# Kiripiro/leaffliction

Hardware: AMD Instinct MI355X
Metric: 224x224 images/sec train (higher is better)
Workload: dtype f32; 1 GPU; leaf_cnn base train step (configs[1]: img 224, batch 256/GPU, fp32, 8 classes, AdamW+clipnorm+EMA, in-model augmentation); per_gpu_batch=256, global_batch=256, img_size=224, parallelism=dp1

## Files before the change

### include/leafhip.h

```cpp
#ifndef LEAFHIP_H
#define LEAFHIP_H

#include <stddef.h>
#include <stdint.h>

#ifdef __cplusplus
extern "C" {
#endif

#define LF_OK 0
#define LF_ERR_INVALID (-1)
#define LF_ERR_LAUNCH (-2)
#define LF_ERR_WORKSPACE (-3)

#define LF_VERSION 100

typedef void* lf_stream_t;

int lf_version(void);
const char* lf_last_error(void);

int lf_copy_rows(void* dst, size_t dst_pitch, const void* src, size_t src_pitch, size_t width, size_t rows, int to_host,
                 lf_stream_t stream);

// ... 296 lines not shown
                        int accumulate, int mask, int* out);
int lf_conv2d_wgrad_bf16_plan(int n, int cin, int h, int w, int cout, int ksize, int* out);

long long lf_conv2d_stats_tiles(int n, int cin, int h, int w, int cout, int ksize);
int lf_conv2d_stats_f32(const float* x, const float* w, float* y, int n, int cin, int h, int wd,
                        int cout, int ksize, const float* in_scale, const float* in_shift,
                        int in_relu, const float* pivot, float* tile_part, size_t tile_part_bytes,
                        lf_stream_t stream, const float* wino_u);

int lf_conv2d_bnbwd_f32(const float* x, const float* w, float* y, int n, int cin, int h, int wd,
                        int cout, int ksize, int accumulate, const float* mask_y,
                        const float* mask_scale, const float* mask_shift, int mask_relu,
                        float* tile_part, size_t tile_part_bytes, lf_stream_t stream, const float* wino_u);

int lf_conv2d_dgrad_weights_f32(const float* w, float* wt, int cin, int ksize, int cout,
                                lf_stream_t stream);

int lf_conv2d_takes_wino_filters(int cin, int h, int wd, int cout, int ksize);
int lf_conv2d_wino_filters_f32(const float* w, float* u, int cin, int cout, int dgrad, lf_stream_t stream);

size_t lf_conv2d_wgrad_workspace(int n, int cin, int h, int wd, int cout, int ksize);
int lf_conv2d_wgrad_f32(const float* x, const float* dy, int n, int cin, int h, int wd, int cout,
                        int ksize, const float* in_scale, const float* in_shift, int in_relu,
                        void* workspace, size_t ws_bytes, lf_stream_t stream);
int lf_conv2d_wgrad_reduce_f32(void* workspace, float* dw, int n, int cin, int h, int wd,
                               int cout, int ksize, float beta, lf_stream_t stream);
int lf_conv2d_wgrad_bn_supported(int n, int cin, int h, int w, int cout, int ksize);
int lf_conv2d_wgrad_bn_f32(const float* x, const float* g, const float* bn_y,
                           const float* alpha_nc, const float* add_nc, const float* coef,
                           int bn_relu, float* dy_out, int n, int cin, int h, int w, int cout,
                           int ksize, const float* in_scale, const float* in_shift, int in_relu,
                           void* workspace, size_t ws_bytes, lf_stream_t stream);

int lf_dwconv3x3_f32(const float* x, const float* w, float* y, int n, int c, int h, int wd,
                     const float* in_scale, const float* in_shift, int in_relu, lf_stream_t stream);
size_t lf_dwconv3x3_bwd_workspace(int n, int c, int h, int wd);
int lf_dwconv3x3_bwd_f32(const float* x, const float* w, const float* dy, float* dx, int accumulate, float* dw,
                         int n, int c, int h, int wd, const float* in_scale, const float* in_shift, int in_relu,
                         void* workspace, size_t ws_bytes, lf_stream_t stream);

int lf_head_distill_fwd_f32(const float* feat, const float* w, const float* b, const float* ytrue,
                            const float* tprobs, float temperature, float alpha, float* probs, float* soft,
                            float* loss, float* kd, int n, int f, int c, lf_stream_t stream);
int lf_head_distill_bwd_f32(const float* feat, const float* w, const float* probs, const float* ytrue,
                            const float* soft, float temperature, float alpha, float* dlogits, float* dfeat,
                            float* dw, float* db, int n, int f, int c, float inv_n, lf_stream_t stream);

int lf_input_stage_f32(const uint8_t* in, float* out, int n, int h, int w, const float* aug4,
                       const float* mean3, const float* denom3, float* means_ws,
                       lf_stream_t stream);

int lf_scale_shift_act_f32(const float* x, float* out, int n, int c, int hw, const float* scale,
                           const float* shift, int relu, lf_stream_t stream);
size_t lf_bn_workspace(int c);
int lf_bn_train_stats_f32(const float* y, int n, int c, int hw, const float* gamma,
                          const float* beta, float* moving_mean, float* moving_var, float momentum,
                          float eps, float* mean, float* invstd, float* scale, float* shift,
                          void* workspace, size_t ws_bytes, lf_stream_t stream);
int lf_bn_train_stats_tiles_f32(const float* tile_part, long long tiles, int n, int c, int hw,
                                const float* gamma, const float* beta, float* moving_mean,
                                float* moving_var, float momentum, float eps, float* mean,
                                float* invstd, float* scale, float* shift, void* workspace,
                                size_t ws_bytes, lf_stream_t stream);
int lf_bn_infer_scale_shift_f32(int c, const float* gamma, const float* beta,
                                const float* moving_mean, const float* moving_var, float eps,
                                float* scale, float* shift, lf_stream_t stream);
// ... 60 lines not shown
```

### leaffliction_amd/_lib.py

```python
from __future__ import annotations

import ctypes as C
import os
from pathlib import Path

_LIB = None

LIB_PATH = Path(__file__).resolve().parent / "libleafhip.so"

c_void_p, c_int, c_size_t, c_u64, c_float, c_double = (
    C.c_void_p, C.c_int, C.c_size_t, C.c_uint64, C.c_float, C.c_double)
P = c_void_p

SIGNATURES = {
    "lf_version": [],
    "lf_last_error": [],
    "lf_pack_hwc_u8_to_nchw_f32": [P, P, c_int, c_int, c_int, P, P, P],
    "lf_hist_u8": [P, P, c_int, c_int, c_int, P],
    "lf_autocontrast_lut": [P, P, P, c_int, P],
    "lf_lut_apply_u8": [P, P, P, c_int, c_int, c_int, P],
    "lf_gather_rows_u8": [P, P, P, c_int, c_size_t, P],
    "lf_flip_u8": [P, P, P, c_int, c_int, c_int, P],
    "lf_noise_wrap_add_u8": [P, P, P, c_size_t, P],
    "lf_add_wrap_u8": [P, P, P, c_size_t, P],
# ... 79 lines not shown
    "lf_canvas_tiles_u8": [P, c_int, c_int, c_int, P, P, c_size_t, c_int, c_int, c_int, P],
    "lf_hist_figure_u8": [P, P, P, c_int, P],
    "lf_conv2d_bf16_stats_tiles": [c_int, c_int, c_int, c_int, c_int, c_int, c_int],
    "lf_conv2d_bf16_train": [P, c_int, P, P, c_int, c_int, c_int, c_int, c_int, c_int, P, P, c_int, c_int, P,
                             c_size_t, P, P, P, P, c_int, P],
    "lf_conv2d_wgrad_bf16_workspace": [c_int, c_int, c_int, c_int, c_int, c_int],
    "lf_conv2d_wgrad_bf16": [P, P, P, P, P, P, c_int, P, P, c_int, c_int, c_int, c_int, c_int, c_int, P, P,
                             c_int, P, c_size_t, P],
    "lf_gap_stats_bf16": [P, P, P, c_int, c_int, c_int, P, P, c_int, P],
    "lf_block_tail_fwd_train_bf16": [P, P, P, P, P, P, P, c_int, P, P, P, c_int, c_int, c_int, c_int, P],
    "lf_block_tail_bwd_bf16": [P, P, P, P, P, P, P, P, P, P, P, c_int, c_int, c_int, c_int, P],
    "lf_bcast_planes_bf16": [P, P, c_int, c_int, c_float, P],
    "lf_cast_f32_bf16": [P, P, c_size_t, P],
    "lf_cast_bf16_f32": [P, P, c_size_t, P],
    "lf_conv2d_variant": [c_int, c_int, c_int, c_int],
    "lf_conv2d_wgrad_variant": [c_int, c_int, c_int, c_int, c_int, c_int],
    "lf_conv2d_plan": [c_int, c_int, c_int, c_int, c_int, c_int, P],
    "lf_conv2d_wgrad_plan": [c_int, c_int, c_int, c_int, c_int, c_int, P],
    "lf_conv2d_bf16_plan": [c_int, c_int, c_int, c_int, c_int, c_int, c_int, c_int, c_int, c_int, c_int, P],
    "lf_conv2d_wgrad_bf16_plan": [c_int, c_int, c_int, c_int, c_int, c_int, P],
    "lf_conv2d_stats_tiles": [c_int, c_int, c_int, c_int, c_int, c_int],
    "lf_conv2d_stats_f32": [P, P, P, c_int, c_int, c_int, c_int, c_int, c_int, P, P, c_int, P, P, c_size_t, P, P],
    "lf_conv2d_bnbwd_f32": [P, P, P, c_int, c_int, c_int, c_int, c_int, c_int, c_int, P, P, P, c_int, P,
                            c_size_t, P, P],
    "lf_conv2d_dgrad_weights_f32": [P, P, c_int, c_int, c_int, P],
    "lf_conv2d_takes_wino_filters": [c_int, c_int, c_int, c_int, c_int],
    "lf_conv2d_wino_filters_f32": [P, P, c_int, c_int, c_int, P],
    "lf_conv2d_wgrad_workspace": [c_int, c_int, c_int, c_int, c_int, c_int],
    "lf_conv2d_wgrad_f32": [P, P, c_int, c_int, c_int, c_int, c_int, c_int, P, P, c_int, P,
                            c_size_t, P],
    "lf_conv2d_wgrad_bn_supported": [c_int, c_int, c_int, c_int, c_int, c_int],
    "lf_conv2d_wgrad_bn_f32": [P, P, P, P, P, P, c_int, P, c_int, c_int, c_int, c_int, c_int, c_int, P, P,
                               c_int, P, c_size_t, P],
    "lf_dwconv3x3_f32": [P, P, P, c_int, c_int, c_int, c_int, P, P, c_int, P],
    "lf_dwconv3x3_bwd_workspace": [c_int, c_int, c_int, c_int],
    "lf_dwconv3x3_bwd_f32": [P, P, P, P, c_int, P, c_int, c_int, c_int, c_int, P, P, c_int, P, c_size_t, P],
    "lf_conv2d_wgrad_reduce_f32": [P, P, c_int, c_int, c_int, c_int, c_int, c_int, c_float, P],
    "lf_input_stage_f32": [P, P, c_int, c_int, c_int, P, P, P, P, P],
    "lf_scale_shift_act_f32": [P, P, c_int, c_int, c_int, P, P, c_int, P],
    "lf_bn_workspace": [c_int],
    "lf_bn_train_stats_f32": [P, c_int, c_int, c_int, P, P, P, P, c_float, c_float, P, P, P, P,
                              P, c_size_t, P],
    "lf_bn_train_stats_tiles_f32": [P, C.c_longlong, c_int, c_int, c_int, P, P, P, P, c_float, c_float, P, P, P, P, P, c_size_t, P],
    "lf_bn_bwd_sums_f32": [P, P, P, P, P, P, P, P, c_int, P, P, P, P, P, P, c_int, c_int, c_int, P,
                           c_size_t, P],
    "lf_bn_bwd_sums_tiles_f32": [P, C.c_longlong, P, P, P, P, P, P, P, P, c_int, c_int, c_int, P,
                                 c_size_t, P],
    "lf_bn_infer_scale_shift_f32": [c_int, P, P, P, P, c_float, P, P, P],
    "lf_bn_bwd_f32": [P, P, P, P, P, P, P, P, c_int, P, P, P, P, P, P, c_int, c_int, c_int, c_int, P,
                      c_size_t, P],
    "lf_gap_f32": [P, P, c_int, c_int, c_int, P, P, c_int, P, P],
    "lf_bcast_planes_f32": [P, P, c_int, c_int, c_float, P],
    "lf_se_fwd_f32": [P, P, P, P, P, P, P, c_int, c_int, c_int, P],
    "lf_se_bwd_workspace": [c_int, c_int, c_int],
    "lf_se_bwd_f32": [P, P, P, P, P, P, P, P, P, P, P, c_int, c_int, c_int, c_float, P, c_size_t, P],
    "lf_block_tail_fwd_f32": [P, P, P, P, P, P, P, c_int, P, P, P, c_int, c_int, c_int, c_int, P],
    "lf_block_tail_bwd_f32": [P, P, P, P, P, P, P, P, P, P, P, c_int, c_int, c_int, c_int, P],
    "lf_head_fwd_f32": [P, P, P, P, P, P, c_int, c_int, c_int, P],
    "lf_head_bwd_f32": [P, P, P, P, P, P, P, P, c_int, c_int, c_int, c_float, P],
    "lf_head_distill_fwd_f32": [P, P, P, P, P, c_float, c_float, P, P, P, P, c_int, c_int, c_int, P],
    "lf_head_distill_bwd_f32": [P, P, P, P, P, c_float, c_float, P, P, P, P, c_int, c_int, c_int, c_float, P],
    "lf_mul_f32": [P, P, P, c_size_t, P],
    "lf_adamw_workspace": [c_int],
    "lf_adamw_step_f32": [P, P, P, P, P, P, P, c_int, C.c_longlong, c_float, c_float, c_float,
                          c_float, c_float, c_float, C.c_longlong, c_float, c_int, P, P, c_size_t, P],
    "lf_ema_update_f32": [P, P, c_size_t, c_float, c_int, P],
}
_RESTYPES = {"lf_last_error": C.c_char_p, "lf_conv2d_wgrad_workspace": c_size_t,
             "lf_dwconv3x3_bwd_workspace": c_size_t,
             "lf_bn_workspace": c_size_t, "lf_se_bwd_workspace": c_size_t,
             "lf_adamw_workspace": c_size_t, "lf_conv2d_stats_tiles": C.c_longlong,
             "lf_blur_saliency_workspace": c_size_t, "lf_inclusive_mask_workspace": c_size_t, "lf_make_mask_workspace": c_size_t, "lf_brown_spots_workspace": c_size_t, "lf_lesion_table_workspace": c_size_t, "lf_canny_workspace": c_size_t, "lf_clahe_workspace": c_size_t,
             "lf_good_features_workspace": c_size_t, "lf_landmarks_workspace": c_size_t,
             "lf_conv2d_bf16_weight_elems": c_size_t,
             "lf_conv2d_bf16_act_mean_workspace": c_size_t,
             "lf_conv2d_bf16_stats_tiles": C.c_longlong, "lf_conv2d_wgrad_bf16_workspace": c_size_t,
             "lf_jpeg_file_bound": c_size_t, "lf_jpeg_scan_aux_offset": c_size_t, "lf_jpeg_scan_aux_offset_ragged": c_size_t, "lf_jpeg_decode_items_workspace": c_size_t, "lf_jpeg_entropy_workspace": c_size_t, "lf_jpeg_wrap_scan": C.c_long, "lf_jpeg_fdct_groups": C.c_long, "lf_jpeg_decode_workspace": c_size_t, "lf_jpeg_write_file": C.c_long, "lf_jpeg_quant_tables": None}


class ResampleItem(C.Structure):
    _fields_ = [("in_off", C.c_int64), ("tile_start", C.c_int64), ("h", C.c_int32), ("w", C.c_int32),
                ("out_index", C.c_int32), ("xtab", C.c_int32), ("ytab", C.c_int32), ("kx", C.c_int32),
                ("ky", C.c_int32), ("reserved", C.c_int32)]


class LeafHipError(RuntimeError):
    pass


def load():
    global _LIB
    if _LIB is not None:
        return _LIB
    import torch
    path = Path(os.environ.get("LEAFHIP_LIB", LIB_PATH))
    if not path.exists():
        raise LeafHipError(
            f"{path} not found: build it with `python -c 'import __graft_entry__ as g; g.build()'` "
            "or `make -C leaffliction_amd/csrc` (there is no CPU fallback)")
    lib = C.CDLL(str(path))
    for name, argtypes in SIGNATURES.items():
# ... 18 lines not shown
```

### leaffliction_amd/csrc/lf_conv.hip

```cpp
#include <type_traits>

#include "lf_common.h"

namespace {

typedef float f32x16 __attribute__((ext_vector_type(16)));
typedef float f32x4 __attribute__((ext_vector_type(4)));

constexpr int kThreads = 256;

typedef float lf_f4 __attribute__((ext_vector_type(4)));
constexpr unsigned kBufOob = 0xffffffffu;
__device__ __forceinline__ __amdgpu_buffer_rsrc_t buf_rsrc(const float* base, unsigned bytes) {
    return __builtin_amdgcn_make_buffer_rsrc(const_cast<float*>(base), 0, bytes, 0x00020000);
}
__device__ __forceinline__ float4 buf_load4(__amdgpu_buffer_rsrc_t r, unsigned off) {
    const lf_f4 v = __builtin_bit_cast(lf_f4, __builtin_amdgcn_raw_buffer_load_b128(r, off, 0, 0));
    return make_float4(v.x, v.y, v.z, v.w);
}
__device__ __forceinline__ float buf_load1(__amdgpu_buffer_rsrc_t r, unsigned off) {
    return __builtin_bit_cast(float, __builtin_amdgcn_raw_buffer_load_b32(r, off, 0, 0));
}

struct ConvArgs {
// ... 733 lines not shown
    if (__all(y2 && lane_full && co0 + CT <= p.cout))
        epilogue(std::true_type{});
    else
        epilogue(std::false_type{});
    if (stats) write_stat_part<WPX, CT>(p, red, t.bz, t.tile, co0, tid);
}

struct WgradArgs {
    const float* x;
    const float* dy;
    float* part;
    const float* in_scale;
    const float* in_shift;
    int n, cin, cout, h, wd;
    int tiles_x, tiles_y, items, items_per_split;
    int in_relu;
    int vec_ok;
    const float* bn_y;
    const float* bn_alpha;
    const float* bn_add;
    const float* bn_coef;
    float* dy_out;
    int bn_relu;
};

__device__ __forceinline__ float bn_dy1(float g, float y, float al, float ad, float c0, float c1,
                                        float c2, float c3, float c4, int relu) {
    float dz = fmaf(g, al, ad);
    if (relu && !(fmaf(y, c0, c1) > 0.f)) dz = 0.f;
    return fmaf(c2, dz, fmaf(c3, y, c4));
}

template <int TW, int TH, int WCI, int WCO, int KSPL>
__global__ __launch_bounds__(kThreads, 4) void wgrad_mfma_kernel(WgradArgs p) {
    static_assert(WCI * WCO * KSPL == 4, "wave decomposition");
    static_assert(TH % KSPL == 0 && TW % 4 == 0, "rows split across waves, float4 rows");
    constexpr int PP = (TW * TH) | 1;
    constexpr int CI_T = 32 * WCI, CO_T = 32 * WCO;
    constexpr int XSZ = CI_T * PP, DSZ = CO_T * PP;
    constexpr int RED = KSPL > 1 ? 1024 : 0;
    constexpr int LDSF = XSZ + DSZ > RED ? XSZ + DSZ : RED;
    constexpr int TW4 = TW / 4;
    constexpr int NXI = CI_T * TH * TW4, XPT = (NXI + kThreads - 1) / kThreads;
    constexpr int NDI = CO_T * TH * TW4, DPT = (NDI + kThreads - 1) / kThreads;
    __shared__ float lds[LDSF];
    float* lx = lds;
    float* ld = lds + XSZ;

    const int tid = threadIdx.x, lane = tid & 63, wid = tid >> 6;
    const int w_ci = wid % WCI, w_co = (wid / WCI) % WCO, w_k = wid / (WCI * WCO);
    const lf::Block3 blk = lf::xcd_split_block3();
    const int ci0 = blk.y * CI_T, co0 = blk.z * CO_T;
    const int khalf = lane >> 5, j = lane & 31;
    const size_t hw = (size_t)p.h * p.wd;
    const unsigned uhw = (unsigned)hw;

    f32x16 acc;
#pragma unroll
    for (int r = 0; r < 16; ++r) acc[r] = 0.f;

    const int abase = (w_ci * 32 + j) * PP + khalf;
    const int bbase = (w_co * 32 + j) * PP + khalf;
    const bool pro = p.in_scale != nullptr;

    auto compute_item = [&]() {
        constexpr int ROWS = TH / KSPL;
#pragma unroll
// ... 202 lines not shown
        }
    }

    if (KSPL > 1) {
        const int q = w_co * WCI + w_ci;
#pragma unroll 1
        for (int k = 1; k < KSPL; ++k) {
#pragma unroll 1
            for (int qq = 0; qq < WCI * WCO; ++qq) {
                __syncthreads();
                if (w_k == k && q == qq) {
#pragma unroll
                    for (int r = 0; r < 16; ++r) lds[r * 64 + lane] = acc[r];
                }
                __syncthreads();
                if (w_k == 0 && q == qq) {
#pragma unroll
                    for (int r = 0; r < 16; ++r) acc[r] += lds[r * 64 + lane];
                }
            }
        }
    }
    if (w_k == 0) {
        float* out = p.part + (size_t)blk.x * p.cin * p.cout;
        const int co = co0 + w_co * 32 + j;
#pragma unroll
        for (int r = 0; r < 16; ++r) {
            const int ci = ci0 + w_ci * 32 + (r & 3) + 8 * (r >> 2) + 4 * khalf;
            if (ci < p.cin && co < p.cout) out[(size_t)ci * p.cout + co] = acc[r];
        }
    }
}


template <int TW, int TH, int WCI, int WCO, int KSPL>
constexpr int wgrad3_lds_floats() {
    const int pp = ((TW + 2) * (TH + 2)) | 1, dp = (TW * TH) | 1;
    const int buf = 32 * WCI * pp + 32 * WCO * dp;
    const int red = KSPL > 1 ? 16 * 1024 : 0;
    const int xch = WCI * WCO * 2 * 3 * 1024;
    const int m = 2 * buf > red ? 2 * buf : red;
    return m > xch ? m : xch;
}

template <int TW, int TH, int WCI, int WCO, int KSPL>
__global__ __launch_bounds__(64 * 2 * WCI * WCO * KSPL, 2) void wgrad3_kernel(WgradArgs p) {
    constexpr int NT = 64 * 2 * WCI * WCO * KSPL;
    constexpr int TWH = TW / 2, NTILE = TWH * (TH / 2), SH = NTILE / KSPL;
    static_assert(TH % 2 == 0 && TW % 4 == 0 && NTILE % KSPL == 0 && SH % 2 == 0,
                  "2x2 tiles split across waves in pairs, float4 rows");
    static_assert(SH % TWH == 0 || TWH % SH == 0, "a K-split share is whole tile rows or part of one");
    constexpr int PW = TW + 2, PH = TH + 2;
    constexpr int PP = (PW * PH) | 1;
    constexpr int DP = (TW * TH) | 1;
    constexpr int CI_T = 32 * WCI, CO_T = 32 * WCO, NQ = WCI * WCO;
    constexpr int XSZ = CI_T * PP, DSZ = CO_T * DP;
    constexpr int BUF = XSZ + DSZ;
    static_assert(wgrad3_lds_floats<TW, TH, WCI, WCO, KSPL>() >= 2 * BUF, "LDS sizing");
    constexpr int TW4 = TW / 4;
    constexpr int NXI = CI_T * PH * TW4, XPT = (NXI + NT - 1) / NT;
    constexpr int NHI = CI_T * PH * 2 * 1, HPT = (NHI + NT - 1) / NT;
    constexpr int NDI = CO_T * TH * TW4, DPT = (NDI + NT - 1) / NT;
    extern __shared__ __attribute__((aligned(16))) float lds[];

    const int tid = threadIdx.x, lane = tid & 63, wid = tid >> 6;
    const int pg = wid & 1, rest = wid >> 1;
// ... 654 lines not shown
        best.tiles_x = (w + 31) / 32;
        best.tiles_y = (h + 7) / 8;
        best.gy = 1;
        best.gz = (cout + 31) / 32;
    } else {
        long long best_cost = -1;
        for (int v = 0; v < (int)(sizeof(kWgVariants) / sizeof(kWgVariants[0])); ++v) {
            const WgVariant& k = kWgVariants[v];
            const long long tx = (w + k.tw - 1) / k.tw, ty = (h + k.th - 1) / k.th;
            const long long gy = (cin + k.ci_t - 1) / k.ci_t, gz = (cout + k.co_t - 1) / k.co_t;
            const long long cost = tx * k.tw * ty * k.th * gy * k.ci_t * gz * k.co_t;
            if (best_cost < 0 || cost < best_cost) {
                best_cost = cost;
                best.variant = v;
                best.tw = k.tw;
                best.tiles_x = (int)tx;
                best.tiles_y = (int)ty;
                best.gy = (int)gy;
                best.gz = (int)gz;
            }
        }
    }
    best.items = n * best.tiles_x * best.tiles_y;
    int splits = (256 * (ksize == 3 && best.variant != kWgSmallCin ? 2 : 3)) / (best.gy * best.gz);
    if (splits < 1) splits = 1;
    if (splits > best.items) splits = best.items;
    best.items_per_split = (best.items + splits - 1) / splits;
    best.splits = (best.items + best.items_per_split - 1) / best.items_per_split;
    return best;
}

inline bool aligned16(const void* p) { return (reinterpret_cast<size_t>(p) & 15) == 0; }

inline int conv_stack(int variant, int n, int cin, int h, int wd, int cout) {
    const FwdVariant& v = kFwdVariants[variant];
    if (variant != 4 || n < 2 || v.th > h) return 1;
    if (h % v.th == 0 || (2 * h) % v.th != 0) return 1;
    if (wd % v.tw != 0 || wd % 4 != 0 || cout % 4 != 0 || cin % 8 != 0) return 1;
    if ((size_t)2 * cin * h * wd >= (1ull << 29) || (size_t)2 * cout * h * wd >= (1ull << 30)) return 1;
    return 2;
}

}

void lf::reduce_slabs(float* part, float* dst, size_t count, int splits, float beta, hipStream_t s) {
    const unsigned gx = lf::stream_grid(count, kThreads, 1024);
    if (slab_stages(splits) == 1) {
        slab_reduce_kernel<<<dim3(gx, 1), kThreads, 0, s>>>(part, dst, count, splits, splits, beta, 1);
    } else {
        const int groups = slab_groups(splits);
        float* stage = part + (size_t)splits * count;
        slab_reduce_kernel<<<dim3(gx, groups), kThreads, 0, s>>>(part, stage, count, splits, kSlabGroup, 0.f, 0);
        slab_reduce_kernel<<<dim3(gx, 1), kThreads, 0, s>>>(stage, dst, count, groups, groups, beta, 1);
    }
}

extern "C" {

int lf_conv2d_wgrad_bn_supported(int n, int cin, int h, int wd, int cout, int ksize);

int lf_conv2d_variant(int h, int wd, int cout, int ksize) {
    int best = 0;
    long long bw = -1;
    for (int v = 0; v < kNumFwd; ++v) {
        const long long c = padded_work(kFwdVariants[v], h, wd, cout);
        const bool better = bw < 0 || c < bw ||
// ... 221 lines not shown
    return wgrad_launch("lf_conv2d_wgrad", x, dy, n, cin, h, wd, cout, ksize, in_scale, in_shift,
                        in_relu, nullptr, nullptr, nullptr, nullptr, 0, nullptr, workspace, ws_bytes,
                        stream);
}

int lf_conv2d_wgrad_bn_supported(int n, int cin, int h, int wd, int cout, int ksize) {
    if (n <= 0 || cin <= 0 || cout <= 0 || h <= 0 || wd <= 0 || (ksize != 3 && ksize != 1)) return 0;
    const WgPlan pl = plan_wgrad(n, cin, cout, h, wd, ksize);
    return (wd % pl.tw == 0) && (wd % 4 == 0);
}

int lf_conv2d_wgrad_bn_f32(const float* x, const float* g, const float* bn_y,
                           const float* alpha_nc, const float* add_nc, const float* coef,
                           int bn_relu, float* dy_out, int n, int cin, int h, int wd, int cout,
                           int ksize, const float* in_scale, const float* in_shift, int in_relu,
                           void* workspace, size_t ws_bytes, lf_stream_t stream) {
    LF_REQUIRE(bn_y, "lf_conv2d_wgrad_bn: null bn_y");
    return wgrad_launch("lf_conv2d_wgrad_bn", x, g, n, cin, h, wd, cout, ksize, in_scale, in_shift,
                        in_relu, bn_y, alpha_nc, add_nc, coef, bn_relu, dy_out, workspace, ws_bytes,
                        stream);
}

int lf_conv2d_wgrad_reduce_f32(void* workspace, float* dw, int n, int cin, int h, int wd, int cout,
                               int ksize, float beta, lf_stream_t stream) {
    LF_REQUIRE(workspace && dw, "lf_conv2d_wgrad_reduce: null buffer");
    LF_REQUIRE(n > 0 && cin > 0 && cout > 0 && h > 0 && wd > 0 && (ksize == 1 || ksize == 3),
               "lf_conv2d_wgrad_reduce: bad dims");
    const WgPlan pl = plan_wgrad(n, cin, cout, h, wd, ksize);
    const size_t count = (size_t)cin * ksize * ksize * cout;
    lf::reduce_slabs(static_cast<float*>(workspace), dw, count, pl.splits, beta, lf::as_stream(stream));
    return lf::check_launch("lf_conv2d_wgrad_reduce");
}

}
```

### leaffliction_amd/model/cnn.py

```python
from __future__ import annotations

import json
import os
import math
import zipfile
from pathlib import Path
from typing import Any, Dict, List, Optional, Tuple

import numpy as np
import torch

from .. import nn, ops

BN_MOMENTUM = 0.99
BN_EPS = 1e-3
NORM_EPS = 1e-7


L2_KINDS = ("w3", "dw", "pw")


def _specs(num_classes: int, widths: List[int], use_se: bool, separable: bool = False):
    def conv3(name, cin, cout):
        if separable:
# ... 528 lines not shown
            h, w = sv[p + "hw"]
            xin, xin_st, y1, y2 = (sv[p + k] for k in ("xin", "xin_st", "y1", "y2"))
            pro = (xin_st[2], xin_st[3], True) if xin_st is not None else (None, None, False)
            s, route, drop = sv[p + "s"], sv[p + "route"], sv[p + "drop"]
            st1, st2 = self.stats[p + "bn1"], self.stats[p + "bn2"]
            gA = B(p + "gA", y1.shape)
            gB = B(p + "gB", y1.shape)
            gC = B(p + "gC", y1.shape)
            ds = B(p + "ds", (n, f), F32) if self.use_se else None
            psum = B(p + "psum", (n, f, 2), F32)
            yp = sv.get(p + "yp")
            psum_p = B(p + "psum_p", (n, f, 2), F32) if yp is not None else None
            nn.block_tail_bwd(dp, route, y2, st2[2], st2[3], drop, gA, ds, psum, yp, psum_p)
            add_nc = None
            if self.use_se:
                dm = B(p + "dm", (n, f), F32)
                nn.se_bwd(ds, sv[p + "m"], sv[p + "z1"], s, P[p + "se.w1"], P[p + "se.w2"], dm,
                          G[p + "se.w1"], G[p + "se.b1"], G[p + "se.w2"], G[p + "se.b2"],
                          dm_scale=1.0 / (h * w))
                add_nc = dm
            if self.separable:
                dp = self._backward_block_separable(sv, i, B, gA, gB, gC, s, add_nc, psum, psum_p)
                continue
            bn_bwd_wgrad(y1, gA, y2, st2, P[p + "bn2.gamma"], G[p + "bn2.gamma"],
                         G[p + "bn2.beta"], True, 3, G[p + "c2.w"], gB, st1[2], st1[3], True,
                         alpha_nc=s, add_nc=add_nc, plane_g=psum,
                         plane_m=sv[p + "msum"] if self.use_se else None)
            tsum = self._dgrad(gB, p + "c2.w", 3, gC, bf16, mask=(y1, st1))
            bn_bwd_wgrad(xin, gC, y1, st1, P[p + "bn1.gamma"], G[p + "bn1.gamma"],
                         G[p + "bn1.beta"], True, 3, G[p + "c1.w"], gB, pro[0], pro[1], pro[2],
                         tile_sums=tsum)
            if cin != f:
                stp = self.stats[p + "bnp"]
                bn_bwd_wgrad(xin, gA, yp, stp, P[p + "bnp.gamma"], G[p + "bnp.gamma"],
                             G[p + "bnp.beta"], False, 1, G[p + "proj.w"], gC, pro[0], pro[1], pro[2],
                             plane_g=psum_p)
                dx = B(p + "dx", xin.shape)
                self._dgrad(gC, p + "proj.w", 1, dx, bf16)
            else:
                dx = gA
            stem_mask = (sv["stem.y"], self.stats["stem.bn"]) if i == 0 else None
            stem_sums = self._dgrad(gB, p + "c1.w", 3, dx, bf16, accumulate=True, mask=stem_mask)
            dp = dx
        if part == 0:
            sv["bwd_dp"] = dp
            return
        if self.separable:
            dys = B("stem.dy", sv["stem.y"].shape)
            self._sep_conv_bwd("stem", sv["x0"], (None, None, False), sv["stem.t"], dp, sv["stem.y"], "stem.bn", dys,
                               B("stem.dt", sv["x0"].shape), None, False)
            return
        bn_bwd_wgrad(sv["x0"], dp, sv["stem.y"], self.stats["stem.bn"], P["stem.bn.gamma"],
                     G["stem.bn.gamma"], G["stem.bn.beta"], True, 3, G["stem.w"], None,
                     tile_sums=stem_sums)

    def _sep_conv_bwd(self, base: str, x, pro, t, g, y, bn: str, dy_buf, dt_buf, dx, accumulate: bool,
                      **sums) -> None:
        P, G = self.p, self.g
        nn.bn_bwd_wgrad(t, g, y, self.stats[bn], P[bn + ".gamma"], G[bn + ".gamma"], G[bn + ".beta"], True, 1,
                        G[base + ".pw"], dy_buf, **sums)
        self._dgrad(dy_buf, base + ".pw", 1, dt_buf, False)
        nn.dwconv3x3_bwd(x, P[base + ".dw"], dt_buf, G[base + ".dw"], dx, accumulate, pro[0], pro[1], pro[2])

    def _backward_block_separable(self, sv, i: int, B, gA, gB, gC, s, add_nc, psum, psum_p):
        P, G = self.p, self.g
        f = self.widths[i]
        cin = self.widths[i - 1] if i > 0 else self.widths[0]
        p = f"s{i}."
        xin, xin_st, y1, y2 = (sv[p + k] for k in ("xin", "xin_st", "y1", "y2"))
        pro = (xin_st[2], xin_st[3], True) if xin_st is not None else (None, None, False)
        st1 = self.stats[p + "bn1"]
# ... 528 lines not shown
```

### leaffliction_amd/nn.py

```python
from __future__ import annotations

import os
from typing import Optional, Tuple

import torch

from . import _lib
from .ops import _chk, _stream

_F32 = torch.float32
_BF16 = torch.bfloat16
_ws_cache = {}
_ws_gen = 0
_NO_FUSED_BN_WGRAD = os.environ.get("LEAFFLICTION_NO_FUSED_BN_WGRAD", "0") == "1"


def _workspace(nbytes: int, device, slot: int = 0) -> torch.Tensor:
    global _ws_gen
    key = (str(device), slot)
    buf = _ws_cache.get(key)
    if buf is None or buf.numel() < nbytes:
        if torch.cuda.is_available() and torch.cuda.is_current_stream_capturing():
            raise RuntimeError("a workspace would have to grow while a HIP graph is being recorded: run the shape "
                               "eagerly first (the warm-up steps size every workspace)")
        buf = torch.empty(max(nbytes, 1 << 20), dtype=torch.uint8, device=device)
        _ws_cache[key] = buf
        _ws_gen += 1
    return buf


def workspace_generation() -> int:
    return _ws_gen


def _ptr(t: Optional[torch.Tensor]):
    return None if t is None else t.data_ptr()


def conv2d_takes_wino_filters(cin: int, h: int, w: int, cout: int, ksize: int) -> bool:
    return bool(_lib.load().lf_conv2d_takes_wino_filters(int(cin), int(h), int(w), int(cout), int(ksize)))


def conv2d_wino_filters(w_iko: torch.Tensor, dgrad: bool = False,
                        out: Optional[torch.Tensor] = None) -> torch.Tensor:
    _chk(w_iko, _F32, "conv2d_wino_filters.w", 3)
    cin, taps, cout = w_iko.shape
    if taps != 9:
# ... 340 lines not shown
              _ptr(in_scale), _ptr(in_shift), 1 if in_relu else 0, ws.data_ptr(), ws.numel(),
              _stream())
    _lib.call("lf_conv2d_wgrad_reduce_f32", ws.data_ptr(), out.data_ptr(), n, cin, h, w, cout,
              ksize, float(beta), _stream())
    return out


def bn_bwd_wgrad(x: torch.Tensor, g: torch.Tensor, y_bn: torch.Tensor, stats: torch.Tensor, gamma,
                 dgamma, dbeta, relu: bool, ksize: int, dw_out: torch.Tensor, dy_out: torch.Tensor,
                 in_scale=None, in_shift=None, in_relu: bool = False, alpha_nc=None, add_nc=None,
                 plane_g=None, plane_m=None, tile_sums=None) -> torch.Tensor:
    who = "bn_bwd_wgrad"
    _chk(x, _F32, f"{who}.x", 4)
    n, cin, h, w, cout = _bn_bwd_wgrad_checks(who, _F32, x, g, y_bn, dy_out, dw_out, ksize, in_scale, in_shift,
                                              alpha_nc, add_nc, plane_g, plane_m)
    lib = _lib.load()
    if _NO_FUSED_BN_WGRAD or not lib.lf_conv2d_wgrad_bn_supported(n, cin, h, w, cout, ksize):
        dy = bn_bwd(g, y_bn, stats, gamma, dgamma, dbeta, relu, alpha_nc=alpha_nc, add_nc=add_nc,
                    out=dy_out, plane_g=plane_g, plane_m=plane_m, tile_sums=tile_sums)
        conv2d_wgrad(x, dy, ksize, in_scale, in_shift, in_relu, out=dw_out)
        return dy_out
    coef, _ = _bn_bwd_coef(who, stats, gamma, dgamma, dbeta, relu, n, cout, h * w, x.device, g, y_bn, alpha_nc,
                           add_nc, plane_g, plane_m, tile_sums)
    ws = _workspace(lib.lf_conv2d_wgrad_workspace(n, cin, h, w, cout, ksize), x.device)
    _lib.call("lf_conv2d_wgrad_bn_f32", x.data_ptr(), g.data_ptr(), y_bn.data_ptr(), _ptr(alpha_nc),
              _ptr(add_nc), coef.data_ptr(), 1 if relu else 0, _ptr(dy_out), n, cin, h, w, cout,
              ksize, _ptr(in_scale), _ptr(in_shift), 1 if in_relu else 0, ws.data_ptr(), ws.numel(),
              _stream())
    _lib.call("lf_conv2d_wgrad_reduce_f32", ws.data_ptr(), dw_out.data_ptr(), n, cin, h, w, cout,
              ksize, 0.0, _stream())
    return dy_out


def _dw_weights(who: str, w_c9: torch.Tensor, c: int) -> None:
    _chk(w_c9, _F32, f"{who}.w", 2)
    if tuple(w_c9.shape) != (c, 9):
        raise ValueError(f"{who}.w: expected [{c},9], got {tuple(w_c9.shape)}")


def dwconv3x3(x: torch.Tensor, w_c9: torch.Tensor, in_scale=None, in_shift=None, in_relu: bool = False,
              out: Optional[torch.Tensor] = None) -> torch.Tensor:
    _chk(x, _F32, "dwconv3x3.x", 4)
    n, c, h, w = x.shape
    _dw_weights("dwconv3x3", w_c9, c)
    _prologue("dwconv3x3", in_scale, in_shift, c)
    out = _act_out("dwconv3x3", out, (n, c, h, w), (_F32,), _F32, x.device)
    _lib.call("lf_dwconv3x3_f32", x.data_ptr(), w_c9.data_ptr(), out.data_ptr(), n, c, h, w, _ptr(in_scale),
              _ptr(in_shift), 1 if in_relu else 0, _stream())
    return out


def dwconv3x3_bwd(x: torch.Tensor, w_c9: torch.Tensor, dy: torch.Tensor, dw_out: torch.Tensor,
                  dx_out: Optional[torch.Tensor] = None, accumulate: bool = False, in_scale=None, in_shift=None,
                  in_relu: bool = False):
    who = "dwconv3x3_bwd"
    _chk(x, _F32, f"{who}.x", 4)
    _chk(dy, _F32, f"{who}.dy", 4)
    n, c, h, w = x.shape
    if dy.shape != x.shape:
        raise ValueError(f"{who}: x and dy must share their shape")
    _dw_weights(who, w_c9, c)
    _dw_weights(f"{who}.dw_out", dw_out, c)
    _prologue(who, in_scale, in_shift, c)
    if dx_out is None and accumulate:
        raise ValueError(f"{who}: accumulate needs dx_out")
    if dx_out is not None:
# ... 288 lines not shown
```

Measured before the change: 6487 images/sec.

## Fuse projection shortcut BN backward, dgrad and wgrad into one MFMA kernel

Adds a fused kernel for the 1x1 projection shortcut's backward pass in fp32. For each pixel tile it applies the BN-backward coefficients to the incoming gradient, computes dx with MFMA against register-held weights, and accumulates the weight gradient, with per-block partial slabs reduced afterwards. This replaces separate BN-bwd+wgrad and dgrad launches, so the intermediate dy is no longer written and re-read. It also lowers the occupancy hint for non-KSPL=2 wgrad variants from 4 to 3 blocks. The fused path only handles cin of 32 or 64 with cout equal to 2*cin, requires no input prologue, and falls back to the old path otherwise.

```diff
diff --git a/include/leafhip.h b/include/leafhip.h
--- a/include/leafhip.h
+++ b/include/leafhip.h
@@ -352,6 +352,14 @@
                            int ksize, const float* in_scale, const float* in_shift, int in_relu,
                            void* workspace, size_t ws_bytes, lf_stream_t stream);
 
+int lf_conv2d_proj_bwd_supported(const float* x, const float* g, const float* bn_y, const float* w,
+                                 const float* dx, int n, int cin, int h, int wd, int cout);
+int lf_conv2d_proj_bwd_plan(int n, int cin, int h, int wd, int cout, int* out);
+size_t lf_conv2d_proj_bwd_workspace(int n, int cin, int h, int wd, int cout);
+int lf_conv2d_proj_bwd_f32(const float* x, const float* g, const float* bn_y, const float* coef, int bn_relu,
+                           const float* w, float* dx, float* dw, int n, int cin, int h, int wd, int cout,
+                           void* workspace, size_t ws_bytes, lf_stream_t stream);
+
 int lf_dwconv3x3_f32(const float* x, const float* w, float* y, int n, int c, int h, int wd,
                      const float* in_scale, const float* in_shift, int in_relu, lf_stream_t stream);
 size_t lf_dwconv3x3_bwd_workspace(int n, int c, int h, int wd);
diff --git a/leaffliction_amd/_lib.py b/leaffliction_amd/_lib.py
--- a/leaffliction_amd/_lib.py
+++ b/leaffliction_amd/_lib.py
@@ -135,6 +135,10 @@
     "lf_conv2d_wgrad_bn_supported": [c_int, c_int, c_int, c_int, c_int, c_int],
     "lf_conv2d_wgrad_bn_f32": [P, P, P, P, P, P, c_int, P, c_int, c_int, c_int, c_int, c_int, c_int, P, P,
                                c_int, P, c_size_t, P],
+    "lf_conv2d_proj_bwd_supported": [P, P, P, P, P, c_int, c_int, c_int, c_int, c_int],
+    "lf_conv2d_proj_bwd_plan": [c_int, c_int, c_int, c_int, c_int, P],
+    "lf_conv2d_proj_bwd_workspace": [c_int, c_int, c_int, c_int, c_int],
+    "lf_conv2d_proj_bwd_f32": [P, P, P, P, c_int, P, P, P, c_int, c_int, c_int, c_int, c_int, P, c_size_t, P],
     "lf_dwconv3x3_f32": [P, P, P, c_int, c_int, c_int, c_int, P, P, c_int, P],
     "lf_dwconv3x3_bwd_workspace": [c_int, c_int, c_int, c_int],
     "lf_dwconv3x3_bwd_f32": [P, P, P, P, c_int, P, c_int, c_int, c_int, c_int, P, P, c_int, P, c_size_t, P],
@@ -170,6 +174,7 @@
     "lf_ema_update_f32": [P, P, c_size_t, c_float, c_int, P],
 }
 _RESTYPES = {"lf_last_error": C.c_char_p, "lf_conv2d_wgrad_workspace": c_size_t,
+             "lf_conv2d_proj_bwd_workspace": c_size_t,
              "lf_dwconv3x3_bwd_workspace": c_size_t,
              "lf_bn_workspace": c_size_t, "lf_se_bwd_workspace": c_size_t,
              "lf_adamw_workspace": c_size_t, "lf_conv2d_stats_tiles": C.c_longlong,
diff --git a/leaffliction_amd/csrc/lf_conv.hip b/leaffliction_amd/csrc/lf_conv.hip
--- a/leaffliction_amd/csrc/lf_conv.hip
+++ b/leaffliction_amd/csrc/lf_conv.hip
@@ -789,7 +789,7 @@
 }
 
 template <int TW, int TH, int WCI, int WCO, int KSPL>
-__global__ __launch_bounds__(kThreads, 4) void wgrad_mfma_kernel(WgradArgs p) {
+__global__ __launch_bounds__(kThreads, KSPL == 2 ? 4 : 3) void wgrad_mfma_kernel(WgradArgs p) {
     static_assert(WCI * WCO * KSPL == 4, "wave decomposition");
     static_assert(TH % KSPL == 0 && TW % 4 == 0, "rows split across waves, float4 rows");
     constexpr int PP = (TW * TH) | 1;
@@ -1058,6 +1058,144 @@
     }
 }
 
+struct ProjBwdArgs {
+    const float* x;
+    const float* g;
+    const float* bn_y;
+    const float* coef;
+    const float* w;
+    float* dx;
+    float* part;
+    int hw, items_per_image, items, items_per_split;
+    int bn_relu;
+};
+
+constexpr int kProjP = 64;
+
+__device__ __forceinline__ void buf_store1(__amdgpu_buffer_rsrc_t r, unsigned off, float v) {
+    __builtin_amdgcn_raw_buffer_store_b32(__builtin_bit_cast(unsigned, v), r, off, 0, 0);
+}
+
+template <int CIB>
+__global__ __launch_bounds__(128 * CIB, 2) void proj_bwd_kernel(ProjBwdArgs p) {
+    constexpr int CIN = 32 * CIB, COUT = 64 * CIB, NT = 128 * CIB;
+    constexpr int P = kProjP, PP = P | 1, P4 = P / 4;
+    constexpr int CSTEP = NT / P4;
+    constexpr int XPT = CIN / CSTEP, DPT = COUT / CSTEP;
+    constexpr int HC = COUT / 2;
+    static_assert(CIN % CSTEP == 0 && COUT % CSTEP == 0 && HC % 4 == 0, "whole float4 slots per thread");
+    __shared__ float lds[(CIN + COUT) * PP + 5 * COUT];
+    float* lx = lds;
+    float* ld = lds + CIN * PP;
+    float* lbn = ld + COUT * PP;
+
+    const int tid = threadIdx.x, lane = tid & 63, wid = tid >> 6;
+    const int khalf = lane >> 5, j = lane & 31;
+    const int cib = wid % CIB, pxb = wid / CIB;
+    const unsigned uhw = (unsigned)p.hw;
+
+    for (int e = tid; e < 5 * COUT; e += NT) lbn[e] = p.coef[e];
+    float wr[HC];
+    {
+        const float4* wp = reinterpret_cast<const float4*>(p.w + (size_t)(cib * 32 + j) * COUT + khalf * HC);
+#pragma unroll
+        for (int q = 0; q < HC / 4; ++q) {
+            const float4 v = wp[q];
+            wr[4 * q] = v.x;
+            wr[4 * q + 1] = v.y;
+            wr[4 * q + 2] = v.z;
+            wr[4 * q + 3] = v.w;
+        }
+    }
+    f32x16 accw[CIB];
+#pragma unroll
+    for (int a = 0; a < CIB; ++a)
+#pragma unroll
+        for (int r = 0; r < 16; ++r) accw[a][r] = 0.f;
+
+    const int c0 = tid / P4, slot = tid % P4;
+    const unsigned goff = 4u * ((unsigned)c0 * uhw + 4u * (unsigned)slot), gstep = 4u * CSTEP * uhw;
+    const int loff = c0 * PP + 4 * slot;
+    const unsigned xbytes = 4u * ((CIN - 1) * uhw + P), dbytes = 4u * ((COUT - 1) * uhw + P);
+    const unsigned soff = 4u * ((unsigned)(cib * 32 + 4 * khalf) * uhw + (unsigned)(pxb * 32 + j));
+
+    float4 xv[XPT], gv[DPT], yv[DPT];
+    auto load_item = [&](int item) {
+        const int n = item / p.items_per_image;
+        const size_t px0 = (size_t)(item - n * p.items_per_image) * P;
+        const __amdgpu_buffer_rsrc_t rx = buf_rsrc(p.x + (size_t)n * CIN * p.hw + px0, xbytes);
+        const __amdgpu_buffer_rsrc_t rg = buf_rsrc(p.g + (size_t)n * COUT * p.hw + px0, dbytes);
+        const __amdgpu_buffer_rsrc_t ry = buf_rsrc(p.bn_y + (size_t)n * COUT * p.hw + px0, dbytes);
+#pragma unroll
+        for (int i = 0; i < XPT; ++i) xv[i] = buf_load4(rx, goff + (unsigned)i * gstep);
+#pragma unroll
+        for (int i = 0; i < DPT; ++i) gv[i] = buf_load4(rg, goff + (unsigned)i * gstep);
+#pragma unroll
+        for (int i = 0; i < DPT; ++i) yv[i] = buf_load4(ry, goff + (unsigned)i * gstep);
+    };
+    auto store_item = [&]() {
+#pragma unroll
+        for (int i = 0; i < XPT; ++i) {
+            float* dst = lx + loff + i * CSTEP * PP;
+            dst[0] = xv[i].x;
+            dst[1] = xv[i].y;
+            dst[2] = xv[i].z;
+            dst[3] = xv[i].w;
+        }
+#pragma unroll
+        for (int i = 0; i < DPT; ++i) {
+            const int c = c0 + i * CSTEP;
+            const float k0 = lbn[c], k1 = lbn[COUT + c], k2 = lbn[2 * COUT + c], k3 = lbn[3 * COUT + c],
+                        k4 = lbn[4 * COUT + c];
+            float* dst = ld + loff + i * CSTEP * PP;
+            dst[0] = bn_dy1(gv[i].x, yv[i].x, 1.f, 0.f, k0, k1, k2, k3, k4, p.bn_relu);
+            dst[1] = bn_dy1(gv[i].y, yv[i].y, 1.f, 0.f, k0, k1, k2, k3, k4, p.bn_relu);
+            dst[2] = bn_dy1(gv[i].z, yv[i].z, 1.f, 0.f, k0, k1, k2, k3, k4, p.bn_relu);
+            dst[3] = bn_dy1(gv[i].w, yv[i].w, 1.f, 0.f, k0, k1, k2, k3, k4, p.bn_relu);
+        }
+    };
+    auto compute_item = [&](int item) {
+        f32x16 accx;
+#pragma unroll
+        for (int r = 0; r < 16; ++r) accx[r] = 0.f;
+        const float* bx = ld + khalf * HC * PP + pxb * 32 + j;
+#pragma unroll
+        for (int s = 0; s < HC; ++s) accx = __builtin_amdgcn_mfma_f32_32x32x2f32(wr[s], bx[s * PP], accx, 0, 0, 0);
+        const int n = item / p.items_per_image;
+        const size_t px0 = (size_t)(item - n * p.items_per_image) * P;
+        const __amdgpu_buffer_rsrc_t rdx = buf_rsrc(p.dx + (size_t)n * CIN * p.hw + px0, xbytes);
+#pragma unroll
+        for (int r = 0; r < 16; ++r) buf_store1(rdx, soff + 4u * (unsigned)((r & 3) + 8 * (r >> 2)) * uhw, accx[r]);
+        const float* bw = ld + (wid * 32 + j) * PP + khalf;
+        const float* aw = lx + j * PP + khalf;
+#pragma unroll 8
+        for (int s = 0; s < P; s += 2) {
+            const float b = bw[s];
+#pragma unroll
+            for (int a = 0; a < CIB; ++a)
+                accw[a] = __builtin_amdgcn_mfma_f32_32x32x2f32(aw[a * 32 * PP + s], b, accw[a], 0, 0, 0);
+        }
+    };
+
+    const int first = blockIdx.x * p.items_per_split;
+    const int last = min(first + p.items_per_split, p.items);
+    if (first < last) load_item(first);
+    for (int item = first; item < last; ++item) {
+        __syncthreads();
+        store_item();
+        __syncthreads();
+        if (item + 1 < last) load_item(item + 1);
+        compute_item(item);
+    }
+
+    float* out = p.part + (size_t)blockIdx.x * CIN * COUT;
+#pragma unroll
+    for (int a = 0; a < CIB; ++a)
+#pragma unroll
+        for (int r = 0; r < 16; ++r)
+            out[(a * 32 + (r & 3) + 8 * (r >> 2) + 4 * khalf) * COUT + wid * 32 + j] = accw[a][r];
+}
+
 
 template <int TW, int TH, int WCI, int WCO, int KSPL>
 constexpr int wgrad3_lds_floats() {
@@ -1778,6 +1916,28 @@
 
 inline bool aligned16(const void* p) { return (reinterpret_cast<size_t>(p) & 15) == 0; }
 
+struct ProjPlan {
+    int cib, items_per_image, items, splits, items_per_split;
+};
+inline bool proj_bwd_shape(int n, int cin, int h, int wd, int cout) {
+    if (n <= 0 || cin <= 0 || cout <= 0 || h <= 0 || wd <= 0) return false;
+    if (cin % 32 != 0 || cout % 32 != 0 || (long long)cin * cout > 8192) return false;
+    if ((cin != 32 && cin != 64) || cout != 2 * cin) return false;
+    const long long hw = (long long)h * wd;
+    return hw % kProjP == 0 && cout * hw < (1ll << 30) && n * (hw / kProjP) < (1ll << 31);
+}
+inline ProjPlan plan_proj_bwd(int n, int cin, int h, int wd) {
+    ProjPlan pl;
+    pl.cib = cin / 32;
+    pl.items_per_image = h * wd / kProjP;
+    pl.items = n * pl.items_per_image;
+    const int resident = 256 * 8 / (2 * pl.cib);
+    const int splits = resident < pl.items ? resident : pl.items;
+    pl.items_per_split = (pl.items + splits - 1) / splits;
+    pl.splits = (pl.items + pl.items_per_split - 1) / pl.items_per_split;
+    return pl;
+}
+
 inline int conv_stack(int variant, int n, int cin, int h, int wd, int cout) {
     const FwdVariant& v = kFwdVariants[variant];
     if (variant != 4 || n < 2 || v.th > h) return 1;
@@ -2065,4 +2225,56 @@
     return lf::check_launch("lf_conv2d_wgrad_reduce");
 }
 
-}
+int lf_conv2d_proj_bwd_supported(const float* x, const float* g, const float* bn_y, const float* w,
+                                 const float* dx, int n, int cin, int h, int wd, int cout) {
+    if (!x || !g || !bn_y || !w || !dx) return 0;
+    if (!aligned16(x) || !aligned16(g) || !aligned16(bn_y) || !aligned16(w) || !aligned16(dx)) return 0;
+    return proj_bwd_shape(n, cin, h, wd, cout) ? 1 : 0;
+}
+
+int lf_conv2d_proj_bwd_plan(int n, int cin, int h, int wd, int cout, int* out) {
+    LF_REQUIRE(out, "lf_conv2d_proj_bwd_plan: null out");
+    LF_REQUIRE(proj_bwd_shape(n, cin, h, wd, cout), "lf_conv2d_proj_bwd_plan: unsupported shape");
+    const ProjPlan pl = plan_proj_bwd(n, cin, h, wd);
+    out[0] = kProjP;
+    out[1] = pl.items_per_split < 3 ? pl.items_per_split : 3;
+    out[2] = lf::slab_stages(pl.splits);
+    return LF_OK;
+}
+
+size_t lf_conv2d_proj_bwd_workspace(int n, int cin, int h, int wd, int cout) {
+    if (!proj_bwd_shape(n, cin, h, wd, cout)) return 0;
+    const ProjPlan pl = plan_proj_bwd(n, cin, h, wd);
+    return ((size_t)pl.splits + lf::slab_groups(pl.splits)) * cin * cout * sizeof(float);
+}
+
+int lf_conv2d_proj_bwd_f32(const float* x, const float* g, const float* bn_y, const float* coef, int bn_relu,
+                           const float* w, float* dx, float* dw, int n, int cin, int h, int wd, int cout,
+                           void* workspace, size_t ws_bytes, lf_stream_t stream) {
+    const char* who = "lf_conv2d_proj_bwd";
+    LF_REQUIRE(x && g && bn_y && coef && w && dx && dw && workspace, "%s: null buffer", who);
+    LF_REQUIRE(lf_conv2d_proj_bwd_supported(x, g, bn_y, w, dx, n, cin, h, wd, cout),
+               "%s: shape/alignment not supported (ask lf_conv2d_proj_bwd_supported first)", who);
+    if (ws_bytes < lf_conv2d_proj_bwd_workspace(n, cin, h, wd, cout)) {
+        lf::set_error("%s: workspace %zu < %zu bytes", who, ws_bytes,
+                      lf_conv2d_proj_bwd_workspace(n, cin, h, wd, cout));
+        return LF_ERR_WORKSPACE;
+    }
+    const ProjPlan pl = plan_proj_bwd(n, cin, h, wd);
+    ProjBwdArgs a;
+    a.x = x; a.g = g; a.bn_y = bn_y; a.coef = coef; a.w = w; a.dx = dx;
+    a.part = static_cast<float*>(workspace);
+    a.hw = h * wd; a.items_per_image = pl.items_per_image; a.items = pl.items;
+    a.items_per_split = pl.items_per_split;
+    a.bn_relu = bn_relu;
+    hipStream_t s = lf::as_stream(stream);
+    if (pl.cib == 1)
+        proj_bwd_kernel<1><<<pl.splits, 128, 0, s>>>(a);
+    else
+        proj_bwd_kernel<2><<<pl.splits, 256, 0, s>>>(a);
+    if (const int rc = lf::check_launch(who)) return rc;
+    lf::reduce_slabs(a.part, dw, (size_t)cin * cout, pl.splits, 0.f, s);
+    return lf::check_launch(who);
+}
+
+}
diff --git a/leaffliction_amd/model/cnn.py b/leaffliction_amd/model/cnn.py
--- a/leaffliction_amd/model/cnn.py
+++ b/leaffliction_amd/model/cnn.py
@@ -584,11 +584,15 @@
                          tile_sums=tsum)
             if cin != f:
                 stp = self.stats[p + "bnp"]
-                bn_bwd_wgrad(xin, gA, yp, stp, P[p + "bnp.gamma"], G[p + "bnp.gamma"],
-                             G[p + "bnp.beta"], False, 1, G[p + "proj.w"], gC, pro[0], pro[1], pro[2],
-                             plane_g=psum_p)
                 dx = B(p + "dx", xin.shape)
-                self._dgrad(gC, p + "proj.w", 1, dx, bf16)
+                if bf16:
+                    bn_bwd_wgrad(xin, gA, yp, stp, P[p + "bnp.gamma"], G[p + "bnp.gamma"],
+                                 G[p + "bnp.beta"], False, 1, G[p + "proj.w"], gC, pro[0], pro[1], pro[2],
+                                 plane_g=psum_p)
+                    self._dgrad(gC, p + "proj.w", 1, dx, bf16)
+                else:
+                    nn.proj_bwd(xin, gA, yp, stp, P[p + "bnp.gamma"], G[p + "bnp.gamma"], G[p + "bnp.beta"],
+                                P[p + "proj.w"], G[p + "proj.w"], dx, gC, pro[0], pro[1], pro[2], plane_g=psum_p)
             else:
                 dx = gA
             stem_mask = (sv["stem.y"], self.stats["stem.bn"]) if i == 0 else None
diff --git a/leaffliction_amd/nn.py b/leaffliction_amd/nn.py
--- a/leaffliction_amd/nn.py
+++ b/leaffliction_amd/nn.py
@@ -13,6 +13,7 @@
 _ws_cache = {}
 _ws_gen = 0
 _NO_FUSED_BN_WGRAD = os.environ.get("LEAFFLICTION_NO_FUSED_BN_WGRAD", "0") == "1"
+_NO_FUSED_PROJ_BWD = os.environ.get("LEAFFLICTION_NO_FUSED_PROJ_BWD", "0") == "1"
 
 
 def _workspace(nbytes: int, device, slot: int = 0) -> torch.Tensor:
@@ -419,6 +420,34 @@
     return dy_out
 
 
+def proj_bwd(x: torch.Tensor, g: torch.Tensor, y_bn: torch.Tensor, stats: torch.Tensor, gamma, dgamma, dbeta,
+             w: torch.Tensor, dw_out: torch.Tensor, dx_out: torch.Tensor, dy_scratch: Optional[torch.Tensor] = None,
+             in_scale=None, in_shift=None, in_relu: bool = False, plane_g=None) -> torch.Tensor:
+    who = "proj_bwd"
+    _chk(x, _F32, f"{who}.x", 4)
+    n, cin, h, wd, cout = _bn_bwd_wgrad_checks(who, _F32, x, g, y_bn, dy_scratch, dw_out, 1, in_scale, in_shift,
+                                               None, None, plane_g, None)
+    _chk(w, _F32, f"{who}.w", 3)
+    _chk(dx_out, _F32, f"{who}.dx_out", 4)
+    if tuple(w.shape) != (cin, 1, cout) or dx_out.shape != x.shape:
+        raise ValueError(f"{who}: shape mismatch")
+    lib = _lib.load()
+    if _NO_FUSED_PROJ_BWD or in_scale is not None or not lib.lf_conv2d_proj_bwd_supported(
+            x.data_ptr(), g.data_ptr(), y_bn.data_ptr(), w.data_ptr(), dx_out.data_ptr(), n, cin, h, wd, cout):
+        if dy_scratch is None:
+            dy_scratch = torch.empty_like(g)
+        bn_bwd_wgrad(x, g, y_bn, stats, gamma, dgamma, dbeta, False, 1, dw_out, dy_scratch, in_scale, in_shift,
+                     in_relu, plane_g=plane_g)
+        return conv2d(dy_scratch, conv2d_dgrad_weights(w, 1), 1, out=dx_out)
+    coef, _ = _bn_bwd_coef(who, stats, gamma, dgamma, dbeta, False, n, cout, h * wd, x.device, g, y_bn,
+                           plane_g=plane_g)
+    ws = _workspace(lib.lf_conv2d_proj_bwd_workspace(n, cin, h, wd, cout), x.device)
+    _lib.call("lf_conv2d_proj_bwd_f32", x.data_ptr(), g.data_ptr(), y_bn.data_ptr(), coef.data_ptr(), 0,
+              w.data_ptr(), dx_out.data_ptr(), dw_out.data_ptr(), n, cin, h, wd, cout, ws.data_ptr(), ws.numel(),
+              _stream())
+    return dx_out
+
+
 def _dw_weights(who: str, w_c9: torch.Tensor, c: int) -> None:
     _chk(w_c9, _F32, f"{who}.w", 2)
     if tuple(w_c9.shape) != (c, 9):
```

New measurement: 6673 images/sec (median of 6 runs). +2.9%, better.
